# aharley/pips

Hardware: AMD Instinct MI355X
Metric: particle-updates/sec (B*S*N*iters/s) at S=8 N=256 368x496 (higher is better)
Workload: dtype f32; 1 GPU; BASELINE configs[1]: B=1/GPU S=8 368x496 N=256 I=6 fp32 stride 8, encoder included, inputs resident in HBM; clips_per_gpu=1, parallelism=clip-sharded x1, collective=none

## Files before the change

### pips_amd/csrc/api.hip

```cpp
#include "common.h"

#include <cstdarg>
#include <cstdio>
#include <cstdlib>
#include <cstring>
#include <mutex>

namespace pips {

static thread_local char g_err[512] = "";

void set_error(const char* fmt, ...) {
    va_list ap;
    va_start(ap, fmt);
    vsnprintf(g_err, sizeof(g_err), fmt, ap);
    va_end(ap);
}

#ifdef PIPS_TUNING
int tune_env(const char* name, int dflt) {
    const char* e = getenv(name);
    return e ? atoi(e) : dflt;
}
#endif
// ... 431 lines not shown
    RUN(launch_inorm_finalize_pivot(ws + P.partial, e.F, tiles, 64, ws + P.st_a, e.st));
    RUN(launch_inorm_apply(ws + P.raw, ws + P.st_a, nullptr, nullptr, ws + P.xa, e.F, H0 * W0, 64, e.st));
    RUN(res_block(e, ci, false, ws + P.xa, H0, W0, ws + P.xb));
    return res_block(e, ci, false, ws + P.xb, H0, W0, ws + P.outs[0]);
}

int enc_front_bf16(const Enc& e, const void* rgbs, int rgb_u8, int H, int W, int& ci) {
    float* ws = e.ws; const EncPlan& P = e.P; const ArenaLayout& A = e.A; hipStream_t st = e.st;
    const int F = e.F, H0 = P.Hs[0], W0 = P.Ws[0];
    int tiles = 0;
    void* xa = ws + P.xa; void* xb = ws + P.xb; void* raw = ws + P.raw; void* mid = ws + P.mid;
    float* st_a = ws + P.st_a; float* st_b = ws + P.st_b;
    RUN(launch_stem_bf16(rgbs, rgb_u8, e.arena + A.conv[0].w, e.arena + A.conv[0].b, xa, ws + P.partial, F, H, W, H0, W0, &tiles, st));
    RUN(launch_inorm_finalize_pivot(ws + P.partial, F, tiles, 64, st_a, st));
    if (conv3x3_c64_takes(H0, W0, F)) {
        RUN(conv_stats(e, ci++, xa, st_a, H0, W0, raw, ws + P.partial, st_b));
        RUN(conv_stats(e, ci++, raw, st_b, H0, W0, mid, ws + P.partial, st_b));
        RUN(launch_inorm_apply_bf16(mid, st_b, xa, st_a, 3, xb, F, H0 * W0, 64, st));
        RUN(conv_stats(e, ci++, xb, nullptr, H0, W0, raw, ws + P.partial, st_a));
        RUN(conv_stats(e, ci++, raw, st_a, H0, W0, mid, ws + P.partial, st_b));
        return launch_inorm_apply_bf16(mid, st_b, xb, nullptr, 1, ws + P.outs[0], F, H0 * W0, 64, st);
    }
    RUN(launch_inorm_apply_bf16(xa, st_a, nullptr, nullptr, 0, xb, F, H0 * W0, 64, st));
    RUN(res_block(e, ci, false, xb, H0, W0, xa));
    return res_block(e, ci, false, xa, H0, W0, ws + P.outs[0]);
}

int encoder_impl(const void* arena_v, const void* rgbs, int F, int H, int W, int stride, int flags, float* pyramid, void* workspace,
                 size_t workspace_bytes, hipStream_t st) {
    PIPS_CHECK_ARG(arena_v && rgbs && pyramid && workspace, "encoder: null pointer");
    RUN(check_geometry(F, H, W, stride));
    const EncPlan P = plan_encoder(F, H, W, stride);
    if (workspace_bytes < P.total * sizeof(float)) {
        set_error("encoder: workspace %zu < %zu bytes", workspace_bytes, P.total * sizeof(float));
        return PIPS_E_WORKSPACE;
    }
    float* ws = (float*)workspace;
    const Enc e = {(const float*)arena_v, arena_layout(), F, ws, P, st, encoder_mode(flags)};
    const bool h = e.mode == BF16;
    const int rgb_u8 = (flags & PIPS_FLAG_RGB_U8) ? 1 : 0;

    int ci = 1;
    RUN(h ? enc_front_bf16(e, rgbs, rgb_u8, H, W, ci) : enc_front_f32(e, rgbs, rgb_u8, H, W, ci));
    const void* x = ws + P.outs[0];
    int Hc = P.Hs[0], Wc = P.Ws[0];
    for (int l = 1; l < 4; ++l) {
        RUN(res_block(e, ci, true, x, Hc, Wc, ws + P.xb));
        Hc = P.Hs[l]; Wc = P.Ws[l];
        RUN(res_block(e, ci, false, ws + P.xb, Hc, Wc, ws + P.outs[l]));
        x = ws + P.outs[l];
    }
    const int ch[4] = {64, 96, 128, 128};
    const int H8 = P.Hs[4], W8 = P.Ws[4];
    for (int l = 0, coff = 0; l < 4; coff += ch[l], ++l)
        RUN(h ? launch_resize_into_bf16(ws + P.outs[l], F, P.Hs[l], P.Ws[l], ch[l], ws + P.cat, H8, W8, 416, coff, st)
              : launch_resize_into(ws + P.outs[l], F, P.Hs[l], P.Ws[l], ch[l], ws + P.cat, H8, W8, 416, coff, st));
    const int i2 = ci++, i3 = ci++;
    RUN(conv_stats(e, i2, ws + P.cat, nullptr, H8, W8, ws + P.raw, ws + P.partial, ws + P.st_a));
    RUN(inorm_apply(e, ws + P.raw, ws + P.st_a, nullptr, nullptr, ws + P.mid, H8 * W8, 256));
    RUN(conv_nhwc(enc_conv(e, i3, ws + P.mid, H8, W8, pyramid, false), st));
    const PyramidView v = pyramid_view(F, H8, W8);
    for (int l = 1; l < PIPS_LEVELS; ++l)
        RUN(launch_avgpool2(pyramid + v.off[l - 1], F, v.lh[l - 1], v.lw[l - 1], PIPS_C, pyramid + v.off[l], st));
    if (h) RUN(launch_pyramid_mirror(pyramid, v.levels, pyramid + v.levels, st));
    return PIPS_OK;
}

enum GatherRoute { GATHER_AUTO, GATHER_DIRECT, GATHER_TILED };

struct GatherCall {
    const float* pyramid; int B, T, R, S, H8, W8;
    const float* ffeats; const float* coords; const float* times; int N;
    const int* win_start; const int* win_dir;
    float* X;
    bool bf16_maps; GatherRoute route;
    void* scratch; size_t scratch_bytes; hipEvent_t* ev;
    hipStream_t st;
};

int mixer_input(const GatherCall& g) {
    PIPS_CHECK_ARG(g.pyramid && g.ffeats && g.coords && g.times && g.X, "mixer_input: null pointer");
    PIPS_CHECK_ARG(g.T >= 1 && g.R >= 1 && g.B > 0 && g.N > 0, "mixer_input: need T, R, B, N >= 1");
    PIPS_CHECK_ARG(g.S >= 1 && g.S <= PIPS_S_MAX, "mixer_input: window length S=%d outside 1..%d", g.S, PIPS_S_MAX);
    const PyramidView v = pyramid_view(g.B * g.R, g.H8, g.W8);
    PIPS_CHECK_ARG(!v.empty(), "mixer_input: map too small");
    const float* mirror = g.pyramid + v.levels;
    const bool can_tile = g.scratch != nullptr && g.win_start == nullptr && g.win_dir == nullptr && g.R == PIPS_S && g.T == g.R &&
                          g.S == PIPS_S && g.scratch_bytes >= tiled_gather_scratch_bytes(g.B, g.N, g.H8, g.W8);
    const bool tiled = g.route == GATHER_AUTO ? tiled_gather_wanted(g.B, g.N, g.H8, g.W8, g.bf16_maps) : g.route == GATHER_TILED;
    if (tiled && can_tile)
        return launch_mixer_input_tiled(g.pyramid, v.off, v.lh, v.lw, g.B, g.R, g.ffeats, g.coords, g.times, g.N, g.X, g.scratch,
                                        g.scratch_bytes, g.st, g.ev,
                                        g.bf16_maps ? reinterpret_cast<const unsigned short*>(mirror) : nullptr);
    PIPS_CHECK_ARG(g.route != GATHER_TILED, "tiled gather needs scratch of %zu bytes, no win_start and 8 frames per clip",
                   tiled_gather_scratch_bytes(g.B, g.N, g.H8, g.W8));
    PIPS_CHECK_ARG(g.win_dir == nullptr || g.win_start != nullptr, "mixer_input: win_dir needs win_start");
    if (g.bf16_maps)
        return launch_mixer_input_bf16maps(mirror, v.off, v.lh, v.lw, g.B, g.R, g.T, g.ffeats, g.coords, g.times, g.N, g.win_start,
                                           g.win_dir, g.X, g.st, g.S);
    return launch_mixer_input(g.pyramid, v.off, v.lh, v.lw, g.B, g.R, g.T, g.ffeats, g.coords, g.times, g.N, g.win_start, g.win_dir,
                              g.X, g.st, g.S);
}

int mixer_input_tiled(GatherCall g, float* ms3_host) {
    PIPS_CHECK_ARG(g.scratch != nullptr, "mixer_input_tiled: null pointer");
    PIPS_CHECK_ARG(g.R == PIPS_S, "mixer_input_tiled: S must be %d", PIPS_S);
    g.route = GATHER_TILED;
    if (ms3_host == nullptr) return mixer_input(g);
    Events ev(4);
    if (!ev.ok()) return PIPS_E_LAUNCH;
    g.ev = ev.ev;
    int rc = mixer_input(g);
    if (rc == PIPS_OK && !ev.wait(3)) rc = PIPS_E_LAUNCH;
    if (rc == PIPS_OK)
        for (int i = 0; i < 3; ++i) ms3_host[i] = ev.elapsed(i, i + 1);
    return rc;
// ... 154 lines not shown
FwdPlan plan_forward(int B, int S, int H, int W, int N, int stride) {
    FwdPlan P;
    Bump b;
    const int F = B * S;
    P.pyramid = b.take(pyramid_view(F, H / stride, W / stride).total());
    P.enc = b.take(plan_encoder(F, H, W, stride).total);
    P.track = b.take(plan_track(B, N, S).total);
    P.total = b.off;
    return P;
}

size_t score_map_workspace_bytes(int B, int S, int H8, int W8) {
    if (B <= 0 || S <= 0 || H8 <= 0 || W8 <= 0) return 0;
    return (size_t)B * S * H8 * W8 * PIPS_C * sizeof(float);
}
int score_map_prepare(const float* pyramid, int B, int S, int H8, int W8, float* U, hipStream_t st) {
    PIPS_CHECK_ARG(pyramid && U && B > 0 && S > 0 && H8 >= 8 && W8 >= 8, "score_map_prepare: bad argument");
    const PyramidView v = pyramid_view(B * S, H8, W8);
    return launch_score_upsum(pyramid, v.off, v.lh, v.lw, B * S, U, st);
}

struct TrackCall {
    const void* arena; const float* pyramid;
    int B, T, R, S, H8, W8;
    const float* xys; const float* coords_init; const float* feat_init;
    const int* win_start; const int* win_dir;
    const float* times; int N, stride, iters, flags;
    void* workspace; size_t workspace_bytes;
    float* out_trajs; float* out_vis; float* out_ffeat0;
    const float* ce_tgt; float* ce_terms; void* ce_ws; size_t ce_ws_bytes;
    hipStream_t st;
};

int track_impl(const TrackCall& c) {
    PIPS_CHECK_ARG(c.arena && c.pyramid && c.xys && c.times && c.workspace && c.out_trajs && c.out_vis, "track: null pointer");
    PIPS_CHECK_ARG(c.B > 0 && c.N > 0 && c.T >= 1 && c.R >= 1 && c.iters >= 0 && c.stride >= 1,
                   "track: need B,N,T,R,stride >= 1 and iters >= 0");
    PIPS_CHECK_ARG(c.S >= 1 && c.S <= PIPS_S_MAX, "track: window length S=%d outside 1..%d", c.S, PIPS_S_MAX);
    PIPS_CHECK_ARG(c.H8 >= 8 && c.W8 >= 8, "track: map %dx%d too small for a 4-level pyramid", c.H8, c.W8);
    PIPS_CHECK_ARG(c.win_dir == nullptr || c.win_start != nullptr, "track: win_dir needs win_start");
    const int B = c.B, N = c.N, S = c.S;
    const TrackPlan P = plan_track(B, N, S);
    if (c.workspace_bytes < P.total * sizeof(float)) {
        set_error("track: workspace %zu < %zu bytes", c.workspace_bytes, P.total * sizeof(float));
        return PIPS_E_WORKSPACE;
    }
    hipStream_t st = c.st;
    const float* arena = (const float*)c.arena;
    float* ws = (float*)c.workspace;
    const int M = B * N * S;
    float* coords = ws + P.coords; float* coords0 = ws + P.coords0; float* ffeats = ws + P.ffeats;
    float* ffeat0 = c.out_ffeat0 != nullptr ? c.out_ffeat0 : ws + P.ffeat0;
    const size_t traj_sz = (size_t)B * S * N * 2;
    RUN(launch_init_coords(c.xys, c.coords_init, B, N, (float)c.stride, coords, coords0, c.out_trajs, st, S));
    if (c.feat_init != nullptr) {
        if (c.feat_init != ffeat0)
            (void)hipMemcpyAsync(ffeat0, c.feat_init, (size_t)B * N * PIPS_C * sizeof(float), hipMemcpyDeviceToDevice, st);
    } else {
        RUN(launch_point_sample_strided(c.pyramid, B, c.R, c.T, c.H8, c.W8, coords, S * 2, N, c.win_start, ffeat0, st));
    }
    RUN(launch_init_ffeats(ffeat0, B * N, ffeats, st, S));
    if (c.ce_tgt != nullptr) {
        PIPS_CHECK_ARG(c.ce_terms && c.ce_ws && c.win_start == nullptr && c.T == S && c.R == c.T,
                       "track: score-map terms need their output and workspace, S frames per clip and no windows");
        if (c.ce_ws_bytes < score_map_workspace_bytes(B, c.T, c.H8, c.W8)) {
            set_error("track: score-map workspace %zu < %zu bytes", c.ce_ws_bytes, score_map_workspace_bytes(B, c.T, c.H8, c.W8));
            return PIPS_E_WORKSPACE;
        }
        RUN(score_map_prepare(c.pyramid, B, c.T, c.H8, c.W8, (float*)c.ce_ws, st));
    }
    if (c.iters == 0)
        RUN(launch_vis_head(arena, ffeats, B, N, c.out_vis, st, S));
    GatherCall g;
    memset(&g, 0, sizeof(g));
    g.pyramid = c.pyramid; g.B = B; g.T = c.T; g.R = c.R; g.S = S; g.H8 = c.H8; g.W8 = c.W8;
    g.ffeats = ffeats; g.coords = coords; g.times = c.times; g.N = N;
    g.win_start = c.win_start; g.win_dir = c.win_dir;
    g.X = ws + P.X;
    g.bf16_maps = (c.flags & PIPS_FLAG_BF16_MAPS) != 0;
    g.route = GATHER_AUTO;
    g.scratch = ws + P.mixer; g.scratch_bytes = mixer_workspace_bytes(M, S);
    g.st = st;
    for (int it = 0; it < c.iters; ++it) {
        if (c.ce_tgt != nullptr)
            RUN(launch_score_terms((const float*)c.ce_ws, B, S, c.H8, c.W8, ffeats, N, c.ce_tgt, c.ce_terms + (size_t)it * M * 2, st));
        RUN(mixer_input(g));
        RUN(mixer_impl(arena, ws + P.X, M, S, mixer_mode(c.flags), ws + P.delta, ws + P.mixer, mixer_workspace_bytes(M, S), st, nullptr));
        RUN(launch_state_update(arena, ws + P.delta, ffeats, coords, coords0, B, N, (float)c.stride,
                                c.out_trajs + (size_t)(it + 1) * traj_sz, it + 1 == c.iters ? c.out_vis : nullptr, st, S));
    }
    PIPS_CHECK_LAUNCH("pips_track");
    return PIPS_OK;
}

TrackCall track_call(const void* arena, const float* pyramid, int B, int T, int H8, int W8, const float* xys, const float* coords_init,
                     const float* feat_init, const int* win_start, const float* times, int N, int stride, int iters, int flags,
                     void* workspace, size_t workspace_bytes, float* out_trajs, float* out_vis, float* out_ffeat0, void* stream) {
    TrackCall c;
    memset(&c, 0, sizeof(c));
    c.arena = arena; c.pyramid = pyramid; c.B = B; c.T = T; c.H8 = H8; c.W8 = W8;
    c.xys = xys; c.coords_init = coords_init; c.feat_init = feat_init; c.win_start = win_start;
    c.times = times; c.N = N; c.stride = stride; c.iters = iters; c.flags = flags;
    c.workspace = workspace; c.workspace_bytes = workspace_bytes;
    c.out_trajs = out_trajs; c.out_vis = out_vis; c.out_ffeat0 = out_ffeat0;
    c.st = (hipStream_t)stream;
    c.R = T; c.S = PIPS_S;
    return c;
}

GatherCall gather_call(const float* pyramid, int B, int frames, int H8, int W8, const float* ffeats, const float* coords,
                       const float* times, int N, float* X, void* stream) {
    GatherCall g;
    memset(&g, 0, sizeof(g));
    g.pyramid = pyramid; g.B = B; g.T = g.R = frames; g.S = PIPS_S; g.H8 = H8; g.W8 = W8;
// ... 354 lines not shown
```

### pips_amd/csrc/common.h

```cpp
#pragma once
#include <hip/hip_runtime.h>
#include <atomic>
#include <stdint.h>
#include <stddef.h>
#include "../../include/pips_hip.h"

namespace pips {

void set_error(const char* fmt, ...);

#define PIPS_CHECK_ARG(cond, ...)                                   \
    do {                                                            \
        if (!(cond)) { ::pips::set_error(__VA_ARGS__); return PIPS_E_ARG; } \
    } while (0)

#define PIPS_CHECK_LAUNCH(what)                                                     \
    do {                                                                            \
        hipError_t e__ = hipGetLastError();                                         \
        if (e__ != hipSuccess) {                                                    \
            ::pips::set_error("%s: %s", what, hipGetErrorString(e__));              \
            return PIPS_E_LAUNCH;                                                   \
        }                                                                           \
    } while (0)

// ... 207 lines not shown
                }
            }
    }
}

int launch_gemm(const GemmArgs& a, hipStream_t st);
int gemm_f32_t4_route(const GemmArgs& a, int* tpb);
int launch_gemm_f32_t4(const GemmArgs& a, int route, int tpb, hipStream_t st);
int launch_conv(const GemmArgs& a, int frames, int* tiles_m, hipStream_t st);
int conv_f32_t4_config(const GemmArgs& a, int frames);
int launch_conv_f32_t4(const GemmArgs& a, int cfg, int frames, int* parts_out, hipStream_t st);
int launch_gemm_bf16(const GemmArgs& a, int a_bf16, int out_bf16, hipStream_t st);
int launch_conv_bf16(const GemmArgs& a, int frames, int* tiles_m, hipStream_t st, int in_bf16 = 0, int out_bf16 = 0);
int launch_conv3x3_c64_bf16(const GemmArgs& a, int frames, int* tiles_m, hipStream_t st, int in_bf16 = 0, int out_bf16 = 0);
bool conv3x3_c64_takes(int H, int W, int frames);
bool conv_c96_t4_takes(const GemmArgs& a, int frames, int in_bf16, int out_bf16);
int launch_conv_c96_t4(const GemmArgs& a, int frames, int* parts_out, hipStream_t st);
int gemm_bf16_asm_route(const GemmArgs& a, int a_bf16, int out_bf16);
bool gemm_bf16_t4_takes(const GemmArgs& a, int a_bf16, int out_bf16);
int launch_gemm_bf16_t4(const GemmArgs& a, hipStream_t st);
bool gemm_bf16_t4up_takes(const GemmArgs& a, int a_bf16, int out_bf16, int* tpb);
int launch_gemm_bf16_t4up(const GemmArgs& a, int tpb, hipStream_t st);
int launch_split_bf16x3(const float* src, size_t n, void* dst, hipStream_t st);
int launch_gemm_x3(const GemmArgs& a, hipStream_t st);
int launch_conv_x3(const GemmArgs& a, int frames, int* tiles_m, hipStream_t st);

struct ConvW { size_t w, b; int cout, cin, k, stride, pad; };
struct MixLayerW { size_t tw0, tb0, tw3, tb3, ln1g, ln1b, ln2g, ln2b, w1, b1, w2, b2; };
struct ArenaLayout {
    ConvW conv[22];
    size_t w_in, b_in;
    MixLayerW mix[PIPS_DEPTH];
    size_t lnf_g, lnf_b, w_head, b_head;
    size_t norm_g, norm_b, w_upd_t, b_upd, w_vis, b_vis;
    size_t total;
    size_t h_w1[PIPS_DEPTH], h_w2[PIPS_DEPTH], h_head, h_conv[22], h_in, total_h;
    size_t t_in, t_w1[PIPS_DEPTH], t_w2[PIPS_DEPTH], t_head, t_conv[22], total_t;
    int S, nout, nout_pad;
    size_t total_all;
};
const ArenaLayout& arena_layout(int S = PIPS_S);

inline int conv_out(int x, int k, int s, int p) { return (x + 2 * p - k) / s + 1; }

int launch_stem(const void* rgbs, int rgb_u8, const float* w, const float* bias, float* out, float* stats,
                int F, int H, int W, int Ho, int Wo, int* tiles_m, hipStream_t st);
int stem_tiles_m(int Ho, int Wo);
int launch_inorm_finalize_pivot(const float* partial, int F, int parts, int C, float* mean_rstd, hipStream_t st);
int launch_inorm_apply(const float* x, const float* stats, const float* res, const float* res_stats,
                       float* y, int F, int HW, int C, hipStream_t st);
int launch_resize_into(const float* src, int F, int Hs, int Ws, int C, float* dst, int Hd, int Wd,
                       int Cdst, int coff, hipStream_t st);
int launch_avgpool2(const float* src, int F, int H, int W, int C, float* dst, hipStream_t st);
int launch_resize_frames(const void* src, int src_u8, int planes, int h, int w, float* dst, int H, int W, hipStream_t st);
int launch_stem_bf16(const void* rgbs, int rgb_u8, const float* w, const float* bias, void* out_bf16, float* stats,
                     int F, int H, int W, int Ho, int Wo, int* tiles_m, hipStream_t st);
int launch_inorm_apply_bf16(const void* x, const float* stats, const void* res, const float* res_stats, int mode,
                            void* y, int F, int HW, int C, hipStream_t st);
int launch_resize_into_bf16(const void* src, int F, int Hs, int Ws, int C, void* dst, int Hd, int Wd, int Cdst, int coff,
                            hipStream_t st);

int launch_point_sample(const float* level0, int B, int S, int H8, int W8, const float* xy, int N,
                        float* out, hipStream_t st);
int launch_point_sample_strided(const float* level0, int B, int S, int T, int H8, int W8, const float* xy,
                                int xy_stride, int N, const int* win_start, float* out, hipStream_t st);
int launch_init_coords(const float* xys, const float* coords_init, int B, int N, float stride,
                       float* coords, float* coords0, float* out_traj0, hipStream_t st, int Sw = PIPS_S);
int launch_init_ffeats(const float* ffeat0, int BN, float* ffeats, hipStream_t st, int Sw = PIPS_S);
int launch_mixer_input(const float* pyramid, const size_t* lvl_off, const int* lvlH, const int* lvlW,
                       int B, int S, int T, const float* ffeats, const float* coords, const float* times,
                       int N, const int* win_start, const int* win_dir, float* X, hipStream_t st, int Sw = PIPS_S);
int launch_mixer_input_bf16maps(const void* mirror, const size_t* lvl_off, const int* lvlH, const int* lvlW, int B, int S,
                                int T, const float* ffeats, const float* coords, const float* times, int N,
                                const int* win_start, const int* win_dir, float* X, hipStream_t st, int Sw = PIPS_S);
int launch_pyramid_mirror(const float* pyramid, size_t floats, void* mirror, hipStream_t st);
int launch_pyramid_append(const float* src, const size_t* src_off, int k, float* dst, const size_t* dst_off, void* dst_mirror,
                          const int* pf8, int R, int T0, hipStream_t st);
size_t tiled_gather_scratch_bytes(int B, int N, int H8, int W8);
bool tiled_gather_wanted(int B, int N, int H8, int W8, bool bf16_maps = false);
int launch_mixer_input_tiled(const float* pyramid, const size_t* lvl_off, const int* lvlH, const int* lvlW, int B,
                             int S, const float* ffeats, const float* coords, const float* times, int N,
                             float* X, void* scratch, size_t scratch_bytes, hipStream_t st, hipEvent_t* ev = nullptr,
                             const unsigned short* mirror = nullptr);
int launch_token_mix(const float* arena, const MixLayerW& L, float* x, float* xn, int particles,
                     hipStream_t st, int xn_bf16 = 0, int Sw = PIPS_S, int x_bf16 = 0);
int launch_ln_mean(const float* x, const float* g, const float* b, float* out, int particles,
                   hipStream_t st, int Sw = PIPS_S, int x_bf16 = 0);
int launch_score_upsum(const float* pyramid, const size_t* lvl_off, const int* lvlH, const int* lvlW, int F, float* U,
                       hipStream_t st);
int launch_score_terms(const float* U, int B, int S, int H8, int W8, const float* ffeats, int N, const float* tgt,
                       float* out, hipStream_t st);
int launch_vis_head(const float* arena, const float* ffeats, int B, int N, float* out_vis, hipStream_t st, int Sw = PIPS_S);
int launch_state_update(const float* arena, const float* delta, float* ffeats, float* coords,
                        const float* coords0, int B, int N, float stride, float* out_traj,
                        float* out_vis, hipStream_t st, int Sw = PIPS_S);

}
```

### pips_amd/csrc/encoder.hip

```cpp
#include "common.h"

namespace pips {

constexpr int STEM_ROWS = 4, STEM_COLS = 64;
constexpr int STEM_TH = 2 * STEM_ROWS + 5, STEM_TW = 136;
constexpr int STEM_STEPS = 3 * 7 * 4;
constexpr int STEM_LDS = (3 * STEM_TH * STEM_TW + STEM_STEPS * 64 * 2) * 4;

template <typename RGB, bool V4>
__global__ __launch_bounds__(256, 2) void stem_conv_kernel(const RGB* __restrict__ rgbs,
                                                           const float* __restrict__ w,
                                                           const float* __restrict__ bias,
                                                           float* __restrict__ out,
                                                           float* __restrict__ stats, int H, int W,
                                                           int Ho, int Wo, int tiles_x, int tiles, int F) {
    extern __shared__ __attribute__((aligned(16))) float stem_sm[];
    float* tile = stem_sm;
    float* wl = stem_sm + 3 * STEM_TH * STEM_TW;
    const int tid = threadIdx.x, lane = tid & 63, wave = tid >> 6;
    const int l31 = lane & 31, half = lane >> 5;
    for (int i = tid; i < STEM_STEPS * 64 * 2; i += 256) {
        const int h = i & 1, n = (i >> 1) & 63, s = i >> 7;
        const int j = s & 3, ck = s >> 2, kw = 2 * j + h - (V4 ? 1 : 0);
        wl[i] = (kw >= 0 && kw < 7) ? w[(ck * 7 + kw) * 64 + n] : 0.f;
// ... 221 lines not shown

template <int MODE>
__global__ __launch_bounds__(256) void inorm_apply_kernel(const float4* __restrict__ x,
                                                          const float2* __restrict__ stats,
                                                          const float4* __restrict__ res,
                                                          const float2* __restrict__ res_stats,
                                                          float4* __restrict__ y, int HW, int C4,
                                                          size_t total4) {
    const size_t per_frame = (size_t)HW * C4;
    for (size_t i = (size_t)blockIdx.x * blockDim.x + threadIdx.x; i < total4;
         i += (size_t)gridDim.x * blockDim.x) {
        const int f = (int)(i / per_frame);
        const int c4 = (int)(i % C4);
        const float2* st = stats + ((size_t)f * C4 + c4) * 4;
        float4 v = x[i];
        float o[4] = {v.x, v.y, v.z, v.w};
#pragma unroll
        for (int k = 0; k < 4; ++k) o[k] = fmaxf((o[k] - st[k].x) * st[k].y, 0.f);
        if (MODE == 1) {
            const float4 r = res[i];
            o[0] = fmaxf(r.x + o[0], 0.f); o[1] = fmaxf(r.y + o[1], 0.f);
            o[2] = fmaxf(r.z + o[2], 0.f); o[3] = fmaxf(r.w + o[3], 0.f);
        } else if (MODE == 2) {
            const float4 r = res[i];
            const float2* rs = res_stats + ((size_t)f * C4 + c4) * 4;
            const float rr[4] = {r.x, r.y, r.z, r.w};
#pragma unroll
            for (int k = 0; k < 4; ++k) o[k] = fmaxf((rr[k] - rs[k].x) * rs[k].y + o[k], 0.f);
        }
        y[i] = make_float4(o[0], o[1], o[2], o[3]);
    }
}

int launch_inorm_apply(const float* x, const float* stats, const float* res, const float* res_stats,
                       float* y, int F, int HW, int C, hipStream_t st) {
    PIPS_CHECK_ARG(C % 4 == 0, "inorm_apply: C %% 4");
    const size_t total4 = (size_t)F * HW * (C / 4);
    const int blocks = (int)((total4 + 255) / 256 < 4096 ? (total4 + 255) / 256 : 4096);
    const float4* x4 = reinterpret_cast<const float4*>(x);
    const float2* s2 = reinterpret_cast<const float2*>(stats);
    const float4* r4 = reinterpret_cast<const float4*>(res);
    const float2* rs2 = reinterpret_cast<const float2*>(res_stats);
    float4* y4 = reinterpret_cast<float4*>(y);
    if (res == nullptr)
        hipLaunchKernelGGL(inorm_apply_kernel<0>, dim3(blocks), dim3(256), 0, st, x4, s2, r4, rs2, y4, HW, C / 4, total4);
    else if (res_stats == nullptr)
        hipLaunchKernelGGL(inorm_apply_kernel<1>, dim3(blocks), dim3(256), 0, st, x4, s2, r4, rs2, y4, HW, C / 4, total4);
    else
        hipLaunchKernelGGL(inorm_apply_kernel<2>, dim3(blocks), dim3(256), 0, st, x4, s2, r4, rs2, y4, HW, C / 4, total4);
    PIPS_CHECK_LAUNCH("inorm_apply_kernel");
    return PIPS_OK;
}

__global__ __launch_bounds__(256) void resize_into_kernel(const float* __restrict__ src, int Hs, int Ws,
                                                          int C4, float4* __restrict__ dst, int Hd,
                                                          int Wd, int Cdst4, int coff4, float sh,
                                                          float sw, size_t total4) {
    for (size_t i = (size_t)blockIdx.x * blockDim.x + threadIdx.x; i < total4;
         i += (size_t)gridDim.x * blockDim.x) {
        const int c4 = (int)(i % C4);
        size_t p = i / C4;
        const int x = (int)(p % Wd); p /= Wd;
        const int y = (int)(p % Hd);
        const int f = (int)(p / Hd);
        int y0, y1, x0, x1;
        float ly0, ly1, lx0, lx1;
        if (Hd == Hs) { y0 = y1 = y; ly0 = 1.f; ly1 = 0.f; }
        else {
            const float r = sh * (float)y;
            y0 = min((int)floorf(r), Hs - 1);
            ly1 = fminf(fmaxf(r - (float)y0, 0.f), 1.f);
            y1 = y0 + (y0 < Hs - 1 ? 1 : 0);
            ly0 = 1.f - ly1;
        }
        if (Wd == Ws) { x0 = x1 = x; lx0 = 1.f; lx1 = 0.f; }
        else {
            const float r = sw * (float)x;
            x0 = min((int)floorf(r), Ws - 1);
            lx1 = fminf(fmaxf(r - (float)x0, 0.f), 1.f);
            x1 = x0 + (x0 < Ws - 1 ? 1 : 0);
            lx0 = 1.f - lx1;
        }
        const float4* s4 = reinterpret_cast<const float4*>(src) + (size_t)f * Hs * Ws * C4 + c4;
        const float4 v00 = s4[((size_t)y0 * Ws + x0) * C4], v01 = s4[((size_t)y0 * Ws + x1) * C4];
        const float4 v10 = s4[((size_t)y1 * Ws + x0) * C4], v11 = s4[((size_t)y1 * Ws + x1) * C4];
        float4 o;
        o.x = ly0 * (lx0 * v00.x + lx1 * v01.x) + ly1 * (lx0 * v10.x + lx1 * v11.x);
        o.y = ly0 * (lx0 * v00.y + lx1 * v01.y) + ly1 * (lx0 * v10.y + lx1 * v11.y);
        o.z = ly0 * (lx0 * v00.z + lx1 * v01.z) + ly1 * (lx0 * v10.z + lx1 * v11.z);
        o.w = ly0 * (lx0 * v00.w + lx1 * v01.w) + ly1 * (lx0 * v10.w + lx1 * v11.w);
        dst[(((size_t)f * Hd + y) * Wd + x) * Cdst4 + coff4 + c4] = o;
    }
}

int launch_resize_into(const float* src, int F, int Hs, int Ws, int C, float* dst, int Hd, int Wd,
                       int Cdst, int coff, hipStream_t st) {
    PIPS_CHECK_ARG(C % 4 == 0 && Cdst % 4 == 0 && coff % 4 == 0, "resize: channel alignment");
    const size_t total4 = (size_t)F * Hd * Wd * (C / 4);
    const int blocks = (int)((total4 + 255) / 256 < 4096 ? (total4 + 255) / 256 : 4096);
    const float sh = Hd > 1 ? (float)(Hs - 1) / (float)(Hd - 1) : 0.f;
    const float sw = Wd > 1 ? (float)(Ws - 1) / (float)(Wd - 1) : 0.f;
    hipLaunchKernelGGL(resize_into_kernel, dim3(blocks), dim3(256), 0, st, src, Hs, Ws, C / 4,
                       reinterpret_cast<float4*>(dst), Hd, Wd, Cdst / 4, coff / 4, sh, sw, total4);
    PIPS_CHECK_LAUNCH("resize_into_kernel");
    return PIPS_OK;
}

__global__ __launch_bounds__(256) void avgpool2_kernel(const float4* __restrict__ src, int H, int W,
                                                       int C4, float4* __restrict__ dst, int Ho, int Wo,
                                                       size_t total4) {
    for (size_t i = (size_t)blockIdx.x * blockDim.x + threadIdx.x; i < total4;
         i += (size_t)gridDim.x * blockDim.x) {
        const int c4 = (int)(i % C4);
        size_t p = i / C4;
        const int x = (int)(p % Wo); p /= Wo;
        const int y = (int)(p % Ho);
        const int f = (int)(p / Ho);
        const float4* s = src + (((size_t)f * H + 2 * y) * W + 2 * x) * C4 + c4;
        const float4 a = s[0], b = s[C4], c = s[(size_t)W * C4], d = s[(size_t)W * C4 + C4];
        float4 o;
        o.x = (((a.x + b.x) + c.x) + d.x) * 0.25f;
        o.y = (((a.y + b.y) + c.y) + d.y) * 0.25f;
        o.z = (((a.z + b.z) + c.z) + d.z) * 0.25f;
        o.w = (((a.w + b.w) + c.w) + d.w) * 0.25f;
        dst[i] = o;
    }
}

int launch_avgpool2(const float* src, int F, int H, int W, int C, float* dst, hipStream_t st) {
    const int Ho = H / 2, Wo = W / 2;
    PIPS_CHECK_ARG(Ho >= 1 && Wo >= 1, "avgpool: map %dx%d too small", H, W);
    const size_t total4 = (size_t)F * Ho * Wo * (C / 4);
    const int blocks = (int)((total4 + 255) / 256 < 4096 ? (total4 + 255) / 256 : 4096);
    hipLaunchKernelGGL(avgpool2_kernel, dim3(blocks), dim3(256), 0, st,
                       reinterpret_cast<const float4*>(src), H, W, C / 4,
                       reinterpret_cast<float4*>(dst), Ho, Wo, total4);
    PIPS_CHECK_LAUNCH("avgpool2_kernel");
    return PIPS_OK;
}

template <typename T>
__global__ __launch_bounds__(256) void resize_frames_kernel(const T* __restrict__ src, int planes, int h, int w,
                                                            float* __restrict__ dst, int H, int W, float sh, float sw) {
    const size_t i = (size_t)blockIdx.x * blockDim.x + threadIdx.x;
    if (i >= (size_t)planes * H * W) return;
    const int x = (int)(i % W), y = (int)((i / W) % H);
    const size_t pl = i / ((size_t)W * H);
    const float fy = fmaxf(__fsub_rn(__fmul_rn(sh, (float)y + 0.5f), 0.5f), 0.f);
    const float fx = fmaxf(__fsub_rn(__fmul_rn(sw, (float)x + 0.5f), 0.5f), 0.f);
    const int y0 = (int)fy, x0 = (int)fx;
    const int y1 = y0 + (y0 < h - 1 ? 1 : 0), x1 = x0 + (x0 < w - 1 ? 1 : 0);
    const float ly1 = fy - (float)y0, lx1 = fx - (float)x0, ly0 = 1.f - ly1, lx0 = 1.f - lx1;
    const T* p = src + pl * (size_t)h * w;
    const float p00 = (float)p[(size_t)y0 * w + x0], p01 = (float)p[(size_t)y0 * w + x1];
    const float p10 = (float)p[(size_t)y1 * w + x0], p11 = (float)p[(size_t)y1 * w + x1];
    const float top = __fadd_rn(__fmul_rn(lx0, p00), __fmul_rn(lx1, p01));
    const float bot = __fadd_rn(__fmul_rn(lx0, p10), __fmul_rn(lx1, p11));
    dst[i] = __fadd_rn(__fmul_rn(ly0, top), __fmul_rn(ly1, bot));
}

int launch_resize_frames(const void* src, int src_u8, int planes, int h, int w, float* dst, int H, int W, hipStream_t st) {
    const size_t total = (size_t)planes * H * W;
    const float sh = (float)h / (float)H, sw = (float)w / (float)W;
    const unsigned blocks = (unsigned)((total + 255) / 256);
    if (src_u8)
        hipLaunchKernelGGL(resize_frames_kernel<unsigned char>, dim3(blocks), dim3(256), 0, st, (const unsigned char*)src,
                           planes, h, w, dst, H, W, sh, sw);
    else
        hipLaunchKernelGGL(resize_frames_kernel<float>, dim3(blocks), dim3(256), 0, st, (const float*)src, planes, h, w, dst,
                           H, W, sh, sw);
    PIPS_CHECK_LAUNCH("resize_frames_kernel");
    return PIPS_OK;
}

}
```

### pips_amd/csrc/track.hip

```cpp
#include "common.h"

namespace pips {

constexpr int S = PIPS_S;
constexpr int C = PIPS_C;


__global__ __launch_bounds__(128) void point_sample_kernel(const float* __restrict__ level0, int S_, int T_,
                                                           int H, int W, const float* __restrict__ xy,
                                                           int xy_stride, int N,
                                                           const int* __restrict__ win_start,
                                                           float* __restrict__ out) {
    const int pn = blockIdx.x;
    const int b = pn / N;
    const float x = xy[(size_t)pn * xy_stride + 0], y = xy[(size_t)pn * xy_stride + 1];
    const float x0f = floorf(x), y0f = floorf(y);
    const float x1f = x0f + 1.f, y1f = y0f + 1.f;
    const int x0 = min(max((int)x0f, 0), W - 1), x1 = min(max((int)x0f + 1, 0), W - 1);
    const int y0 = min(max((int)y0f, 0), H - 1), y1 = min(max((int)y0f + 1, 0), H - 1);
    const float w00 = __fmul_rn(x1f - x, y1f - y), w01 = __fmul_rn(x - x0f, y1f - y);
    const float w10 = __fmul_rn(x1f - x, y - y0f), w11 = __fmul_rn(x - x0f, y - y0f);
    const int f_first = win_start != nullptr ? ring_slot(min(max(win_start[pn], 0), T_ - 1), S_) : 0;
    const float* f0 = level0 + ((size_t)b * S_ + f_first) * H * W * C;
    const int c = threadIdx.x;
    const float v00 = f0[((size_t)y0 * W + x0) * C + c], v01 = f0[((size_t)y0 * W + x1) * C + c];
    const float v10 = f0[((size_t)y1 * W + x0) * C + c], v11 = f0[((size_t)y1 * W + x1) * C + c];
    float o = __fadd_rn(__fmul_rn(w00, v00), __fmul_rn(w01, v01));
    o = __fadd_rn(o, __fmul_rn(w10, v10));
    o = __fadd_rn(o, __fmul_rn(w11, v11));
    out[(size_t)pn * C + c] = o;
}

int launch_point_sample_strided(const float* level0, int B, int S_, int T_, int H8, int W8, const float* xy,
                                int xy_stride, int N, const int* win_start, float* out, hipStream_t st) {
    hipLaunchKernelGGL(point_sample_kernel, dim3(B * N), dim3(128), 0, st, level0, S_, T_, H8, W8, xy,
                       xy_stride, N, win_start, out);
    PIPS_CHECK_LAUNCH("point_sample_kernel");
    return PIPS_OK;
}

int launch_point_sample(const float* level0, int B, int S_, int H8, int W8, const float* xy, int N,
                        float* out, hipStream_t st) {
    return launch_point_sample_strided(level0, B, S_, S_, H8, W8, xy, 2, N, nullptr, out, st);
}

__global__ void init_coords_kernel(const float* __restrict__ xys, const float* __restrict__ coords_init,
                                   int B, int N, int Sw, float stride, float* __restrict__ coords,
                                   float* __restrict__ coords0, float* __restrict__ out_traj0) {
    const int i = blockIdx.x * blockDim.x + threadIdx.x;
    if (i >= B * N * Sw) return;
    const int s = i % Sw, pn = i / Sw, n = pn % N, b = pn / N;
    float x, y;
    if (coords_init != nullptr) {
        const float* p = coords_init + (((size_t)b * Sw + s) * N + n) * 2;
        x = p[0] / stride; y = p[1] / stride;
    } else {
        x = xys[(size_t)pn * 2 + 0] / stride; y = xys[(size_t)pn * 2 + 1] / stride;
    }
    coords[(size_t)i * 2 + 0] = x; coords[(size_t)i * 2 + 1] = y;
    coords0[(size_t)i * 2 + 0] = x; coords0[(size_t)i * 2 + 1] = y;
    float* o = out_traj0 + (((size_t)b * Sw + s) * N + n) * 2;
    o[0] = x * stride; o[1] = y * stride;
}

__global__ void init_ffeats_kernel(const float4* __restrict__ ffeat0, int BN, int Sw, float4* __restrict__ ffeats) {
    const size_t i = (size_t)blockIdx.x * blockDim.x + threadIdx.x;
    if (i >= (size_t)BN * Sw * (C / 4)) return;
    const size_t pn = i / ((size_t)Sw * (C / 4));
    ffeats[i] = ffeat0[pn * (C / 4) + (i % (C / 4))];
}

int launch_init_coords(const float* xys, const float* coords_init, int B, int N, float stride,
                       float* coords, float* coords0, float* out_traj0, hipStream_t st, int Sw) {
    const int total = B * N * Sw;
    hipLaunchKernelGGL(init_coords_kernel, dim3(cdiv(total, 256)), dim3(256), 0, st, xys, coords_init, B,
                       N, Sw, stride, coords, coords0, out_traj0);
    PIPS_CHECK_LAUNCH("init_coords_kernel");
    return PIPS_OK;
}

int launch_init_ffeats(const float* ffeat0, int BN, float* ffeats, hipStream_t st, int Sw) {
    const size_t total = (size_t)BN * Sw * (C / 4);
    hipLaunchKernelGGL(init_ffeats_kernel, dim3((unsigned)((total + 255) / 256)), dim3(256), 0, st,
                       reinterpret_cast<const float4*>(ffeat0), BN, Sw, reinterpret_cast<float4*>(ffeats));
    PIPS_CHECK_LAUNCH("init_ffeats_kernel");
    return PIPS_OK;
}

struct LevelTable {
    size_t off[PIPS_LEVELS];
    int H[PIPS_LEVELS], W[PIPS_LEVELS];
};

template <int SCT>
__global__ __launch_bounds__(256) __attribute__((amdgpu_waves_per_eu(2, 4))) void mixer_input_kernel(const float* __restrict__ pyramid,
                                                          LevelTable lv, int S_, int T_, int Srt,
                                                          const float* __restrict__ ffeats,
                                                          const float* __restrict__ coords,
                                                          const float* __restrict__ times, int N,
                                                          const int* __restrict__ win_start,
                                                          const int* __restrict__ win_dir,
                                                          float* __restrict__ X) {
    __shared__ float Dw[PIPS_LEVELS][64];
    const int S = SCT ? SCT : Srt;
    const int m = blockIdx.x;
    const int s = m % S, pn = m / S;
    const int b = pn / N;
    int fstart = 0, dir = 1;
    if (win_start != nullptr) {
        fstart = win_start[pn];
        if (win_dir != nullptr) dir = win_dir[pn] < 0 ? -1 : 1;
    }
    const int frame = b * S_ + ring_slot(min(max(fstart + dir * s, 0), T_ - 1), S_);
    const int tid = threadIdx.x, lane = tid & 63;
    const int lvl = __builtin_amdgcn_readfirstlane(tid >> 6);
    const float cxm = coords[(size_t)m * 2 + 0], cym = coords[(size_t)m * 2 + 1];
    float* xrow = X + (size_t)m * PIPS_KIN_PAD;
    const float* ff = ffeats + (size_t)m * C;

    {
        const int H = lv.H[lvl], W = lv.W[lvl];
        const float inv = 1.0f / (float)(1 << lvl);
// ... 1077 lines not shown
```

Baseline: 1.392 million particle-updates/s.

## Fuse encoder resize/concat, pyramid pooling, and track setup launches

Replaces the four per-level resize_into launches with one kernel that uses blockIdx.z to select the level, and the three chained avgpool2 launches with one kernel that computes levels 1-3 directly from level 0. It also merges init_coords, point_sample and init_ffeats into a single per-point setup kernel. The aim is to cut kernel launch overhead and serial dependencies on a small workload. In exchange, the direct pooling rereads level 0 redundantly (up to 64 loads per level-3 output), and the bf16 path stays unfused.

```diff
diff --git a/pips_amd/csrc/api.hip b/pips_amd/csrc/api.hip
--- a/pips_amd/csrc/api.hip
+++ b/pips_amd/csrc/api.hip
@@ -507,16 +507,20 @@
     }
     const int ch[4] = {64, 96, 128, 128};
     const int H8 = P.Hs[4], W8 = P.Ws[4];
-    for (int l = 0, coff = 0; l < 4; coff += ch[l], ++l)
-        RUN(h ? launch_resize_into_bf16(ws + P.outs[l], F, P.Hs[l], P.Ws[l], ch[l], ws + P.cat, H8, W8, 416, coff, st)
-              : launch_resize_into(ws + P.outs[l], F, P.Hs[l], P.Ws[l], ch[l], ws + P.cat, H8, W8, 416, coff, st));
+    if (h) {
+        for (int l = 0, coff = 0; l < 4; coff += ch[l], ++l)
+            RUN(launch_resize_into_bf16(ws + P.outs[l], F, P.Hs[l], P.Ws[l], ch[l], ws + P.cat, H8, W8, 416, coff, st));
+    } else {
+        const float* srcs[4] = {ws + P.outs[0], ws + P.outs[1], ws + P.outs[2], ws + P.outs[3]};
+        RUN(launch_resize_cat4(srcs, P.Hs, P.Ws, ch, F, ws + P.cat, H8, W8, 416, st));
+    }
     const int i2 = ci++, i3 = ci++;
     RUN(conv_stats(e, i2, ws + P.cat, nullptr, H8, W8, ws + P.raw, ws + P.partial, ws + P.st_a));
     RUN(inorm_apply(e, ws + P.raw, ws + P.st_a, nullptr, nullptr, ws + P.mid, H8 * W8, 256));
     RUN(conv_nhwc(enc_conv(e, i3, ws + P.mid, H8, W8, pyramid, false), st));
     const PyramidView v = pyramid_view(F, H8, W8);
-    for (int l = 1; l < PIPS_LEVELS; ++l)
-        RUN(launch_avgpool2(pyramid + v.off[l - 1], F, v.lh[l - 1], v.lw[l - 1], PIPS_C, pyramid + v.off[l], st));
+    static_assert(PIPS_LEVELS == 4, "launch_avgpool_pyramid writes levels 1..3");
+    RUN(launch_avgpool_pyramid(pyramid, v.off, v.lh, v.lw, F, PIPS_C, st));
     if (h) RUN(launch_pyramid_mirror(pyramid, v.levels, pyramid + v.levels, st));
     return PIPS_OK;
 }
@@ -777,14 +781,15 @@
     float* coords = ws + P.coords; float* coords0 = ws + P.coords0; float* ffeats = ws + P.ffeats;
     float* ffeat0 = c.out_ffeat0 != nullptr ? c.out_ffeat0 : ws + P.ffeat0;
     const size_t traj_sz = (size_t)B * S * N * 2;
-    RUN(launch_init_coords(c.xys, c.coords_init, B, N, (float)c.stride, coords, coords0, c.out_trajs, st, S));
     if (c.feat_init != nullptr) {
+        RUN(launch_init_coords(c.xys, c.coords_init, B, N, (float)c.stride, coords, coords0, c.out_trajs, st, S));
         if (c.feat_init != ffeat0)
             (void)hipMemcpyAsync(ffeat0, c.feat_init, (size_t)B * N * PIPS_C * sizeof(float), hipMemcpyDeviceToDevice, st);
+        RUN(launch_init_ffeats(ffeat0, B * N, ffeats, st, S));
     } else {
-        RUN(launch_point_sample_strided(c.pyramid, B, c.R, c.T, c.H8, c.W8, coords, S * 2, N, c.win_start, ffeat0, st));
-    }
-    RUN(launch_init_ffeats(ffeat0, B * N, ffeats, st, S));
+        RUN(launch_track_setup(c.xys, c.coords_init, B, N, (float)c.stride, coords, coords0, c.out_trajs, c.pyramid, c.R, c.T, c.H8,
+                               c.W8, c.win_start, ffeat0, ffeats, st, S));
+    }
     if (c.ce_tgt != nullptr) {
         PIPS_CHECK_ARG(c.ce_terms && c.ce_ws && c.win_start == nullptr && c.T == S && c.R == c.T,
                        "track: score-map terms need their output and workspace, S frames per clip and no windows");
diff --git a/pips_amd/csrc/common.h b/pips_amd/csrc/common.h
--- a/pips_amd/csrc/common.h
+++ b/pips_amd/csrc/common.h
@@ -283,6 +283,9 @@
 int launch_resize_into(const float* src, int F, int Hs, int Ws, int C, float* dst, int Hd, int Wd,
                        int Cdst, int coff, hipStream_t st);
 int launch_avgpool2(const float* src, int F, int H, int W, int C, float* dst, hipStream_t st);
+int launch_resize_cat4(const float* const* src, const int* Hs, const int* Ws, const int* C, int F, float* dst, int Hd, int Wd,
+                       int Cdst, hipStream_t st);
+int launch_avgpool_pyramid(float* pyramid, const size_t* off, const int* lh, const int* lw, int F, int C, hipStream_t st);
 int launch_resize_frames(const void* src, int src_u8, int planes, int h, int w, float* dst, int H, int W, hipStream_t st);
 int launch_stem_bf16(const void* rgbs, int rgb_u8, const float* w, const float* bias, void* out_bf16, float* stats,
                      int F, int H, int W, int Ho, int Wo, int* tiles_m, hipStream_t st);
@@ -298,6 +301,9 @@
 int launch_init_coords(const float* xys, const float* coords_init, int B, int N, float stride,
                        float* coords, float* coords0, float* out_traj0, hipStream_t st, int Sw = PIPS_S);
 int launch_init_ffeats(const float* ffeat0, int BN, float* ffeats, hipStream_t st, int Sw = PIPS_S);
+int launch_track_setup(const float* xys, const float* coords_init, int B, int N, float stride, float* coords, float* coords0,
+                       float* out_traj0, const float* level0, int S, int T, int H8, int W8, const int* win_start, float* ffeat0,
+                       float* ffeats, hipStream_t st, int Sw = PIPS_S);
 int launch_mixer_input(const float* pyramid, const size_t* lvl_off, const int* lvlH, const int* lvlW,
                        int B, int S, int T, const float* ffeats, const float* coords, const float* times,
                        int N, const int* win_start, const int* win_dir, float* X, hipStream_t st, int Sw = PIPS_S);
diff --git a/pips_amd/csrc/encoder.hip b/pips_amd/csrc/encoder.hip
--- a/pips_amd/csrc/encoder.hip
+++ b/pips_amd/csrc/encoder.hip
@@ -297,10 +297,10 @@
     return PIPS_OK;
 }
 
-__global__ __launch_bounds__(256) void resize_into_kernel(const float* __restrict__ src, int Hs, int Ws,
-                                                          int C4, float4* __restrict__ dst, int Hd,
-                                                          int Wd, int Cdst4, int coff4, float sh,
-                                                          float sw, size_t total4) {
+__device__ __forceinline__ void resize_into_body(const float* __restrict__ src, int Hs, int Ws,
+                                                 int C4, float4* __restrict__ dst, int Hd,
+                                                 int Wd, int Cdst4, int coff4, float sh,
+                                                 float sw, size_t total4) {
     for (size_t i = (size_t)blockIdx.x * blockDim.x + threadIdx.x; i < total4;
          i += (size_t)gridDim.x * blockDim.x) {
         const int c4 = (int)(i % C4);
@@ -338,6 +338,44 @@
     }
 }
 
+__global__ __launch_bounds__(256) void resize_into_kernel(const float* __restrict__ src, int Hs, int Ws,
+                                                          int C4, float4* __restrict__ dst, int Hd,
+                                                          int Wd, int Cdst4, int coff4, float sh,
+                                                          float sw, size_t total4) {
+    resize_into_body(src, Hs, Ws, C4, dst, Hd, Wd, Cdst4, coff4, sh, sw, total4);
+}
+
+struct ResizeCat {
+    const float* src[4];
+    int Hs[4], Ws[4], C4[4], coff4[4];
+    float sh[4], sw[4];
+};
+__global__ __launch_bounds__(256) void resize_cat_kernel(ResizeCat rc, int F, float4* __restrict__ dst, int Hd, int Wd,
+                                                         int Cdst4) {
+    const int l = blockIdx.z;
+    resize_into_body(rc.src[l], rc.Hs[l], rc.Ws[l], rc.C4[l], dst, Hd, Wd, Cdst4, rc.coff4[l], rc.sh[l], rc.sw[l],
+                     (size_t)F * Hd * Wd * rc.C4[l]);
+}
+
+int launch_resize_cat4(const float* const* src, const int* Hs, const int* Ws, const int* C, int F, float* dst, int Hd, int Wd,
+                       int Cdst, hipStream_t st) {
+    ResizeCat rc;
+    size_t most = 0;
+    for (int l = 0, coff = 0; l < 4; coff += C[l], ++l) {
+        PIPS_CHECK_ARG(C[l] % 4 == 0 && Cdst % 4 == 0, "resize: channel alignment");
+        rc.src[l] = src[l]; rc.Hs[l] = Hs[l]; rc.Ws[l] = Ws[l]; rc.C4[l] = C[l] / 4; rc.coff4[l] = coff / 4;
+        rc.sh[l] = Hd > 1 ? (float)(Hs[l] - 1) / (float)(Hd - 1) : 0.f;
+        rc.sw[l] = Wd > 1 ? (float)(Ws[l] - 1) / (float)(Wd - 1) : 0.f;
+        const size_t total4 = (size_t)F * Hd * Wd * (C[l] / 4);
+        most = most > total4 ? most : total4;
+    }
+    const int blocks = (int)((most + 255) / 256 < 4096 ? (most + 255) / 256 : 4096);
+    hipLaunchKernelGGL(resize_cat_kernel, dim3(blocks, 1, 4), dim3(256), 0, st, rc, F, reinterpret_cast<float4*>(dst), Hd, Wd,
+                       Cdst / 4);
+    PIPS_CHECK_LAUNCH("resize_cat_kernel");
+    return PIPS_OK;
+}
+
 int launch_resize_into(const float* src, int F, int Hs, int Ws, int C, float* dst, int Hd, int Wd,
                        int Cdst, int coff, hipStream_t st) {
     PIPS_CHECK_ARG(C % 4 == 0 && Cdst % 4 == 0 && coff % 4 == 0, "resize: channel alignment");
@@ -351,6 +389,14 @@
     return PIPS_OK;
 }
 
+__device__ __forceinline__ float4 avg4(const float4 a, const float4 b, const float4 c, const float4 d) {
+    float4 o;
+    o.x = (((a.x + b.x) + c.x) + d.x) * 0.25f;
+    o.y = (((a.y + b.y) + c.y) + d.y) * 0.25f;
+    o.z = (((a.z + b.z) + c.z) + d.z) * 0.25f;
+    o.w = (((a.w + b.w) + c.w) + d.w) * 0.25f;
+    return o;
+}
 __global__ __launch_bounds__(256) void avgpool2_kernel(const float4* __restrict__ src, int H, int W,
                                                        int C4, float4* __restrict__ dst, int Ho, int Wo,
                                                        size_t total4) {
@@ -362,14 +408,59 @@
         const int y = (int)(p % Ho);
         const int f = (int)(p / Ho);
         const float4* s = src + (((size_t)f * H + 2 * y) * W + 2 * x) * C4 + c4;
-        const float4 a = s[0], b = s[C4], c = s[(size_t)W * C4], d = s[(size_t)W * C4 + C4];
-        float4 o;
-        o.x = (((a.x + b.x) + c.x) + d.x) * 0.25f;
-        o.y = (((a.y + b.y) + c.y) + d.y) * 0.25f;
-        o.z = (((a.z + b.z) + c.z) + d.z) * 0.25f;
-        o.w = (((a.w + b.w) + c.w) + d.w) * 0.25f;
-        dst[i] = o;
-    }
+        dst[i] = avg4(s[0], s[C4], s[(size_t)W * C4], s[(size_t)W * C4 + C4]);
+    }
+}
+
+template <int L>
+__device__ __forceinline__ float4 pool_from0(const float4* __restrict__ f0, int W0, int C4, int y, int x) {
+    if constexpr (L == 0) {
+        return f0[((size_t)y * W0 + x) * C4];
+    } else {
+        const float4 a = pool_from0<L - 1>(f0, W0, C4, 2 * y, 2 * x), b = pool_from0<L - 1>(f0, W0, C4, 2 * y, 2 * x + 1);
+        const float4 c = pool_from0<L - 1>(f0, W0, C4, 2 * y + 1, 2 * x), d = pool_from0<L - 1>(f0, W0, C4, 2 * y + 1, 2 * x + 1);
+        return avg4(a, b, c, d);
+    }
+}
+
+struct PoolLevels { size_t off[4]; int H[4], W[4]; };
+
+__global__ __launch_bounds__(256) void avgpool_pyramid_kernel(const float4* __restrict__ l0, PoolLevels pl, int F, int C4,
+                                                              float4* __restrict__ base, size_t n1, size_t n2, size_t n3) {
+    size_t i = (size_t)blockIdx.x * blockDim.x + threadIdx.x;
+    int lvl;
+    if (i < n3) lvl = 3;
+    else if (i < n3 + n2) { lvl = 2; i -= n3; }
+    else if (i < n3 + n2 + n1) { lvl = 1; i -= n3 + n2; }
+    else return;
+    const int Ho = pl.H[lvl], Wo = pl.W[lvl];
+    const int c4 = (int)(i % C4);
+    size_t p = i / C4;
+    const int x = (int)(p % Wo); p /= Wo;
+    const int y = (int)(p % Ho);
+    const int f = (int)(p / Ho);
+    const float4* f0 = l0 + (size_t)f * pl.H[0] * pl.W[0] * C4 + c4;
+    const float4 o = lvl == 1 ? pool_from0<1>(f0, pl.W[0], C4, y, x)
+                   : lvl == 2 ? pool_from0<2>(f0, pl.W[0], C4, y, x) : pool_from0<3>(f0, pl.W[0], C4, y, x);
+    base[pl.off[lvl] + i] = o;
+}
+
+int launch_avgpool_pyramid(float* pyramid, const size_t* off, const int* lh, const int* lw, int F, int C, hipStream_t st) {
+    PoolLevels pl;
+    size_t n[4];
+    for (int l = 0; l < 4; ++l) {
+        PIPS_CHECK_ARG(lh[l] >= 1 && lw[l] >= 1 && (l == 0 || (lh[l] == lh[l - 1] / 2 && lw[l] == lw[l - 1] / 2)),
+                       "avgpool pyramid: level %d is %dx%d", l, lh[l], lw[l]);
+        PIPS_CHECK_ARG(off[l] % 4 == 0, "avgpool pyramid: level alignment");
+        pl.off[l] = off[l] / 4; pl.H[l] = lh[l]; pl.W[l] = lw[l];
+        n[l] = (size_t)F * lh[l] * lw[l] * (C / 4);
+    }
+    const size_t total = n[1] + n[2] + n[3];
+    hipLaunchKernelGGL(avgpool_pyramid_kernel, dim3((unsigned)((total + 255) / 256)), dim3(256), 0, st,
+                       reinterpret_cast<const float4*>(pyramid + off[0]), pl, F, C / 4, reinterpret_cast<float4*>(pyramid),
+                       n[1], n[2], n[3]);
+    PIPS_CHECK_LAUNCH("avgpool_pyramid_kernel");
+    return PIPS_OK;
 }
 
 int launch_avgpool2(const float* src, int F, int H, int W, int C, float* dst, hipStream_t st) {
diff --git a/pips_amd/csrc/track.hip b/pips_amd/csrc/track.hip
--- a/pips_amd/csrc/track.hip
+++ b/pips_amd/csrc/track.hip
@@ -5,6 +5,24 @@
 constexpr int S = PIPS_S;
 constexpr int C = PIPS_C;
 
+
+__device__ __forceinline__ float point_sample_at(const float* __restrict__ level0, int S_, int T_, int H, int W, float x, float y,
+                                                 int b, int pn, const int* __restrict__ win_start, int c) {
+    const float x0f = floorf(x), y0f = floorf(y);
+    const float x1f = x0f + 1.f, y1f = y0f + 1.f;
+    const int x0 = min(max((int)x0f, 0), W - 1), x1 = min(max((int)x0f + 1, 0), W - 1);
+    const int y0 = min(max((int)y0f, 0), H - 1), y1 = min(max((int)y0f + 1, 0), H - 1);
+    const float w00 = __fmul_rn(x1f - x, y1f - y), w01 = __fmul_rn(x - x0f, y1f - y);
+    const float w10 = __fmul_rn(x1f - x, y - y0f), w11 = __fmul_rn(x - x0f, y - y0f);
+    const int f_first = win_start != nullptr ? ring_slot(min(max(win_start[pn], 0), T_ - 1), S_) : 0;
+    const float* f0 = level0 + ((size_t)b * S_ + f_first) * H * W * C;
+    const float v00 = f0[((size_t)y0 * W + x0) * C + c], v01 = f0[((size_t)y0 * W + x1) * C + c];
+    const float v10 = f0[((size_t)y1 * W + x0) * C + c], v11 = f0[((size_t)y1 * W + x1) * C + c];
+    float o = __fadd_rn(__fmul_rn(w00, v00), __fmul_rn(w01, v01));
+    o = __fadd_rn(o, __fmul_rn(w10, v10));
+    o = __fadd_rn(o, __fmul_rn(w11, v11));
+    return o;
+}
 
 __global__ __launch_bounds__(128) void point_sample_kernel(const float* __restrict__ level0, int S_, int T_,
                                                            int H, int W, const float* __restrict__ xy,
@@ -14,21 +32,7 @@
     const int pn = blockIdx.x;
     const int b = pn / N;
     const float x = xy[(size_t)pn * xy_stride + 0], y = xy[(size_t)pn * xy_stride + 1];
-    const float x0f = floorf(x), y0f = floorf(y);
-    const float x1f = x0f + 1.f, y1f = y0f + 1.f;
-    const int x0 = min(max((int)x0f, 0), W - 1), x1 = min(max((int)x0f + 1, 0), W - 1);
-    const int y0 = min(max((int)y0f, 0), H - 1), y1 = min(max((int)y0f + 1, 0), H - 1);
-    const float w00 = __fmul_rn(x1f - x, y1f - y), w01 = __fmul_rn(x - x0f, y1f - y);
-    const float w10 = __fmul_rn(x1f - x, y - y0f), w11 = __fmul_rn(x - x0f, y - y0f);
-    const int f_first = win_start != nullptr ? ring_slot(min(max(win_start[pn], 0), T_ - 1), S_) : 0;
-    const float* f0 = level0 + ((size_t)b * S_ + f_first) * H * W * C;
-    const int c = threadIdx.x;
-    const float v00 = f0[((size_t)y0 * W + x0) * C + c], v01 = f0[((size_t)y0 * W + x1) * C + c];
-    const float v10 = f0[((size_t)y1 * W + x0) * C + c], v11 = f0[((size_t)y1 * W + x1) * C + c];
-    float o = __fadd_rn(__fmul_rn(w00, v00), __fmul_rn(w01, v01));
-    o = __fadd_rn(o, __fmul_rn(w10, v10));
-    o = __fadd_rn(o, __fmul_rn(w11, v11));
-    out[(size_t)pn * C + c] = o;
+    out[(size_t)pn * C + threadIdx.x] = point_sample_at(level0, S_, T_, H, W, x, y, b, pn, win_start, threadIdx.x);
 }
 
 int launch_point_sample_strided(const float* level0, int B, int S_, int T_, int H8, int W8, const float* xy,
@@ -42,6 +46,16 @@
 int launch_point_sample(const float* level0, int B, int S_, int H8, int W8, const float* xy, int N,
                         float* out, hipStream_t st) {
     return launch_point_sample_strided(level0, B, S_, S_, H8, W8, xy, 2, N, nullptr, out, st);
+}
+
+__device__ __forceinline__ void init_coord(const float* __restrict__ xys, const float* __restrict__ coords_init, int b, int n,
+                                           int pn, int s, int Sw, int N, float stride, float& x, float& y) {
+    if (coords_init != nullptr) {
+        const float* p = coords_init + (((size_t)b * Sw + s) * N + n) * 2;
+        x = p[0] / stride; y = p[1] / stride;
+    } else {
+        x = xys[(size_t)pn * 2 + 0] / stride; y = xys[(size_t)pn * 2 + 1] / stride;
+    }
 }
 
 __global__ void init_coords_kernel(const float* __restrict__ xys, const float* __restrict__ coords_init,
@@ -51,12 +65,7 @@
     if (i >= B * N * Sw) return;
     const int s = i % Sw, pn = i / Sw, n = pn % N, b = pn / N;
     float x, y;
-    if (coords_init != nullptr) {
-        const float* p = coords_init + (((size_t)b * Sw + s) * N + n) * 2;
-        x = p[0] / stride; y = p[1] / stride;
-    } else {
-        x = xys[(size_t)pn * 2 + 0] / stride; y = xys[(size_t)pn * 2 + 1] / stride;
-    }
+    init_coord(xys, coords_init, b, n, pn, s, Sw, N, stride, x, y);
     coords[(size_t)i * 2 + 0] = x; coords[(size_t)i * 2 + 1] = y;
     coords0[(size_t)i * 2 + 0] = x; coords0[(size_t)i * 2 + 1] = y;
     float* o = out_traj0 + (((size_t)b * Sw + s) * N + n) * 2;
@@ -68,6 +77,40 @@
     if (i >= (size_t)BN * Sw * (C / 4)) return;
     const size_t pn = i / ((size_t)Sw * (C / 4));
     ffeats[i] = ffeat0[pn * (C / 4) + (i % (C / 4))];
+}
+
+__global__ __launch_bounds__(128) void track_setup_kernel(const float* __restrict__ xys, const float* __restrict__ coords_init,
+                                                          int N, int Sw, float stride, float* __restrict__ coords,
+                                                          float* __restrict__ coords0, float* __restrict__ out_traj0,
+                                                          const float* __restrict__ level0, int S_, int T_, int H, int W,
+                                                          const int* __restrict__ win_start, float* __restrict__ ffeat0,
+                                                          float* __restrict__ ffeats) {
+    const int pn = blockIdx.x, b = pn / N, n = pn - b * N;
+    if ((int)threadIdx.x < Sw) {
+        const int s = threadIdx.x;
+        const size_t i = (size_t)pn * Sw + s;
+        float cx, cy;
+        init_coord(xys, coords_init, b, n, pn, s, Sw, N, stride, cx, cy);
+        coords[i * 2 + 0] = cx; coords[i * 2 + 1] = cy;
+        coords0[i * 2 + 0] = cx; coords0[i * 2 + 1] = cy;
+        float* o = out_traj0 + (((size_t)b * Sw + s) * N + n) * 2;
+        o[0] = cx * stride; o[1] = cy * stride;
+    }
+    float x, y;
+    init_coord(xys, coords_init, b, n, pn, 0, Sw, N, stride, x, y);
+    const float o = point_sample_at(level0, S_, T_, H, W, x, y, b, pn, win_start, threadIdx.x);
+    ffeat0[(size_t)pn * C + threadIdx.x] = o;
+    for (int s = 0; s < Sw; ++s) ffeats[((size_t)pn * Sw + s) * C + threadIdx.x] = o;
+}
+
+int launch_track_setup(const float* xys, const float* coords_init, int B, int N, float stride, float* coords, float* coords0,
+                       float* out_traj0, const float* level0, int S_, int T_, int H8, int W8, const int* win_start, float* ffeat0,
+                       float* ffeats, hipStream_t st, int Sw) {
+    PIPS_CHECK_ARG(Sw >= 1 && Sw <= 128, "track setup: window length %d", Sw);
+    hipLaunchKernelGGL(track_setup_kernel, dim3(B * N), dim3(128), 0, st, xys, coords_init, N, Sw, stride, coords, coords0,
+                       out_traj0, level0, S_, T_, H8, W8, win_start, ffeat0, ffeats);
+    PIPS_CHECK_LAUNCH("track_setup_kernel");
+    return PIPS_OK;
 }
 
 int launch_init_coords(const float* xys, const float* coords_init, int B, int N, float stride,
```

Measured after the change: 1.391 million particle-updates/s. No clear change (-0.1%).
